# DegardinBruno/Kinetic-GAN

Hardware: AMD Instinct MI355X
Metric: G+D train-step samples/sec, NTU (N,3,64,25) bs=64 at 1/2/4/8 MI355X (higher is better)
Workload: dtype f32; 1 GPU; ntu shapes (N,3,64,25), 60 classes, mlp4, G+D WGAN-GP iteration, 64 samples/GPU; global_batch=64, parallelism=dp1, launch=hipgraph

## Files before the change

include/kgan_hip.h:

```cpp
#ifndef KGAN_HIP_H
#define KGAN_HIP_H

#include <stdint.h>

#ifdef __cplusplus
extern "C" {
#endif

#define KG_ABI_VERSION 9

enum { KG_ACT_NONE = 0, KG_ACT_LRELU = 1, KG_ACT_TANH = 2 };
enum { KG_TAP_TIME = 0,
       KG_TAP_CHANBLOCK = 1  };

int         kg_abi_version(void);
const char* kg_arch(void);
const char* kg_last_error(void);
void        kg_reload_env(void);

typedef struct KgConvGroup {
    const float* x;  int64_t x_sN, x_sC;
    int32_t Cin, T_in, V_in;
    int32_t x_lead;
    const int32_t* vmap;
// ... 58 lines not shown
typedef struct KgWgradReduceJob {
    const float* ws;  float* dw;
    int64_t w_sT, w_sO, w_sI;
    int32_t taps, M, Cin, splits, accumulate;
} KgWgradReduceJob;
#define KG_WGRAD_REDUCE_MAX_JOBS 24
typedef struct KgWgradReduceJobs {
    int32_t njobs;
    KgWgradReduceJob job[KG_WGRAD_REDUCE_MAX_JOBS];
} KgWgradReduceJobs;
int     kg_wgrad_reduce_many(const KgWgradReduceJobs* jobs, void* stream);

int64_t kg_wgrad_many_workspace_bytes(const KgWgradArgs* jobs, int32_t njobs);
int     kg_wgrad_many(const KgWgradArgs* jobs, int32_t njobs, float* ws, int64_t ws_bytes, void* stream);
int     kg_wgrad_many_plan(const KgWgradArgs* jobs, int32_t njobs, int32_t* variant, int32_t* splits);

typedef struct KgAggArgs {
    int32_t N, C, K, V, W;
    int32_t T;
    int32_t rep;
    const float* a;
    const float* x;  int64_t x_sN, x_sC;
    const float* y;  int64_t y_sN, y_sC;
    float* out;  int64_t o_sN, o_sC;
    float* ws;  int64_t ws_bytes;
    int32_t a_transposed;
    int32_t defer_sum;
    const float* res;  int64_t r_sN, r_sC;  int32_t r_T, r_V, r_tstride;  const int32_t* r_inv;
    const float* mask;  int64_t m_sN, m_sC;  float slope;
} KgAggArgs;
// ... 723 lines not shown
```

kinetic-gan_amd/_native.py:

```python
from __future__ import annotations

import ctypes as C
import os
from typing import NamedTuple, Optional, Sequence, Tuple

import torch

_PKG = os.path.dirname(os.path.abspath(__file__))
LIB_PATH = os.environ.get("KG_LIB") or os.path.join(_PKG, "libkgan_hip.so")

ACT_NONE, ACT_LRELU, ACT_TANH = 0, 1, 2
ABI_VERSION = 9
TAP_TIME, TAP_CHANBLOCK = 0, 1

c_f32p = C.c_void_p
c_i32p = C.c_void_p


class _ConvGroup(C.Structure):
    _fields_ = [("x", c_f32p), ("x_sN", C.c_int64), ("x_sC", C.c_int64),
                ("Cin", C.c_int32), ("T_in", C.c_int32), ("V_in", C.c_int32),
                ("x_lead", C.c_int32),
                ("vmap", c_i32p),
                ("w", c_f32p), ("w_sT", C.c_int64), ("w_sO", C.c_int64), ("w_sI", C.c_int64),
# ... 38 lines not shown
class _WgradReduceJob(C.Structure):
    _fields_ = [("ws", c_f32p), ("dw", c_f32p), ("w_sT", C.c_int64), ("w_sO", C.c_int64), ("w_sI", C.c_int64),
                ("taps", C.c_int32), ("M", C.c_int32), ("Cin", C.c_int32), ("splits", C.c_int32),
                ("accumulate", C.c_int32)]


WGRAD_REDUCE_MAX_JOBS = 24
WGRAD_TILE_128x128, WGRAD_TILE_64x64, WGRAD_TILE_64x32, WGRAD_TILE_32x64, WGRAD_TILE_32x32 = 0, 1, 2, 3, 4
WGRAD_TILE_NAMES = {WGRAD_TILE_128x128: "128x128", WGRAD_TILE_64x64: "64x64", WGRAD_TILE_64x32: "64x32",
                    WGRAD_TILE_32x64: "32x64", WGRAD_TILE_32x32: "32x32"}
WGRAD_MAX_SPLITS = 128


class _WgradReduceJobs(C.Structure):
    _fields_ = [("njobs", C.c_int32), ("job", _WgradReduceJob * WGRAD_REDUCE_MAX_JOBS)]


class _AggArgs(C.Structure):
    _fields_ = [("N", C.c_int32), ("C", C.c_int32), ("K", C.c_int32), ("V", C.c_int32), ("W", C.c_int32),
                ("T", C.c_int32), ("rep", C.c_int32),
                ("a", c_f32p),
                ("x", c_f32p), ("x_sN", C.c_int64), ("x_sC", C.c_int64),
                ("y", c_f32p), ("y_sN", C.c_int64), ("y_sC", C.c_int64),
                ("out", c_f32p), ("o_sN", C.c_int64), ("o_sC", C.c_int64),
                ("ws", c_f32p), ("ws_bytes", C.c_int64), ("a_transposed", C.c_int32), ("defer_sum", C.c_int32),
                ("res", c_f32p), ("r_sN", C.c_int64), ("r_sC", C.c_int64), ("r_T", C.c_int32), ("r_V", C.c_int32),
                ("r_tstride", C.c_int32), ("r_inv", c_i32p),
                ("mask", c_f32p), ("m_sN", C.c_int64), ("m_sC", C.c_int64), ("slope", C.c_float)]


# ... 481 lines not shown
    "kg_peak_copy": (C.c_int, [C.c_void_p, C.c_void_p, C.c_int64, C.c_void_p]),
    "kg_conv_workspace_bytes": (C.c_int64, [C.POINTER(_ConvArgs)]),
    "kg_conv_plan_info": (C.c_int, [C.POINTER(_ConvArgs), C.POINTER(C.c_int32), C.POINTER(C.c_int32)]),
    "kg_conv": (C.c_int, [C.POINTER(_ConvArgs), C.c_void_p]),
    "kg_conv_pack_bytes": (C.c_int64, [C.POINTER(_ConvArgs)]),
    "kg_conv_pack": (C.c_int, [C.POINTER(_ConvArgs), C.c_void_p, C.c_int64, C.c_void_p]),
    "kg_conv_many": (C.c_int, [C.POINTER(_ConvArgs), C.c_int32, C.c_void_p]),
    "kg_conv_many_plan": (C.c_int, [C.POINTER(_ConvArgs), C.c_int32, C.POINTER(C.c_int32)]),
    "kg_wgrad_workspace_bytes": (C.c_int64, [C.POINTER(_WgradArgs)]),
    "kg_wgrad": (C.c_int, [C.POINTER(_WgradArgs), C.c_void_p]),
    "kg_wgrad_plan_info": (C.c_int, [C.POINTER(_WgradArgs), C.POINTER(C.c_int32), C.POINTER(C.c_int32)]),
    "kg_wgrad_reduce_many": (C.c_int, [C.POINTER(_WgradReduceJobs), C.c_void_p]),
    "kg_wgrad_many_workspace_bytes": (C.c_int64, [C.POINTER(_WgradArgs), C.c_int32]),
    "kg_wgrad_many": (C.c_int, [C.POINTER(_WgradArgs), C.c_int32, C.c_void_p, C.c_int64, C.c_void_p]),
    "kg_wgrad_many_plan": (C.c_int, [C.POINTER(_WgradArgs), C.c_int32, C.POINTER(C.c_int32), C.POINTER(C.c_int32)]),
    "kg_aggconv_supported": (C.c_int, [C.POINTER(_AggConvArgs)]),
    "kg_aggconv": (C.c_int, [C.POINTER(_AggConvArgs), C.c_void_p]),
    "kg_aggconv_plan_info": (C.c_int, [C.POINTER(_AggConvArgs), C.c_int32, C.POINTER(_AggConvPlanInfo)]),
    "kg_agg_plan_info": (C.c_int, [C.POINTER(_AggArgs), C.c_int32, C.POINTER(_AggPlanInfo)]),
    "kg_agg_outer_many_plan": (C.c_int, [C.POINTER(_AggArgs), C.c_int32, C.POINTER(C.c_int32), C.POINTER(C.c_int32)]),
    "kg_agg_expand": (C.c_int, [C.POINTER(_AggArgs), C.c_void_p]),
    "kg_agg_reduce": (C.c_int, [C.POINTER(_AggArgs), C.c_void_p]),
    "kg_agg_outer_workspace_bytes": (C.c_int64, [C.POINTER(_AggArgs)]),
    "kg_agg_outer": (C.c_int, [C.POINTER(_AggArgs), C.c_void_p]),
    "kg_agg_outer_slabs": (C.c_int, [C.POINTER(_AggArgs)]),
    "kg_agg_outer_many": (C.c_int, [C.POINTER(_AggArgs), C.c_int32, C.c_void_p]),
    "kg_agg_outer_sum_many": (C.c_int, [C.POINTER(_OuterSumJobs), C.c_void_p]),
    "kg_gen_expand": (C.c_int, [C.POINTER(_GenArgs), C.c_void_p]),
    "kg_gen_fold": (C.c_int, [C.POINTER(_GenArgs), C.c_void_p]),
    "kg_gen_adj_finish": (C.c_int, [C.POINTER(_GenAdjJob), C.c_int32, C.c_void_p]),
# ... 81 lines not shown
    "kg_cls_head_workspace_bytes": (C.c_int64, [C.POINTER(_ClsHeadArgs)]),
    "kg_cls_head_fwd": (C.c_int, [C.POINTER(_ClsHeadArgs), C.c_void_p]),
    "kg_cls_head_bwd": (C.c_int, [C.POINTER(_ClsHeadArgs), C.c_void_p]),
    "kg_cls_head_wgrad": (C.c_int, [C.POINTER(_ClsHeadArgs), C.c_void_p]),
    "kg_cls_scores": (C.c_int, [C.POINTER(_ClsScoresArgs), C.c_void_p]),
    "kg_kin_desc_workspace_bytes": (C.c_int64, [C.POINTER(_KinDescArgs)]),
    "kg_kin_desc_lds_bytes": (C.c_int64, [C.POINTER(_KinDescArgs)]),
    "kg_kin_desc": (C.c_int, [C.POINTER(_KinDescArgs), C.c_void_p]),
    "kg_kin_desc_sets_workspace_bytes": (C.c_int64, [C.POINTER(_KinDescSetsArgs)]),
    "kg_kin_desc_sets_lds_bytes": (C.c_int64, [C.POINTER(_KinDescSetsArgs)]),
    "kg_kin_desc_sets": (C.c_int, [C.POINTER(_KinDescSetsArgs), C.c_void_p]),
    "kg_kin_scores_lds_bytes": (C.c_int64, [C.POINTER(_KinScoresArgs)]),
    "kg_kin_scores": (C.c_int, [C.POINTER(_KinScoresArgs), C.c_void_p]),
}

_lib = None


def load_library():
    global _lib
    if _lib is not None:
        return _lib
    if not os.path.exists(LIB_PATH):
        raise RuntimeError(
            f"{LIB_PATH} is missing: run `python -c 'import __graft_entry__ as g; g.build()'` "
            "(hipcc --offload-arch=gfx950). There is no CPU fallback for the st_gcn path.")
    lib = C.CDLL(LIB_PATH)
    for name, (res, args) in EXPORTS.items():
        fn = getattr(lib, name)
        fn.restype = res
        fn.argtypes = args
    if lib.kg_abi_version() != ABI_VERSION:
        raise RuntimeError("libkgan_hip.so ABI version mismatch")
    _lib = lib
    return lib


def _check(rc: int, what: str):
    if rc != 0:
        msg = load_library().kg_last_error().decode()
        raise RuntimeError(f"{what} failed (rc={rc}): {msg}")


# ... 312 lines not shown
    a = _wgrad_args(g, x, Cin, taps, tap_mode, t_stride, vmap, wv, dw, accumulate, extra, keep)
    ws = _workspace("kg_wgrad_workspace_bytes", a, g.device)
    if last_wgrad_plan is not None:
        v, ns = C.c_int32(), C.c_int32()
        _check(lib.kg_wgrad_plan_info(C.byref(a), C.byref(v), C.byref(ns)), "kg_wgrad_plan_info")
        last_wgrad_plan[:] = [(v.value, ns.value)]
    if defer is not None:
        a.defer_reduce = 1
        per = taps * a.M * Cin
        defer.append(dict(ws=ws, dw=dw, w_sT=wv.sT, w_sO=wv.sO, w_sI=wv.sI, taps=taps, M=a.M, Cin=Cin,
                          splits=max(1, ws.numel() // per), accumulate=int(accumulate)))
    _check(lib.kg_wgrad(C.byref(a), _stream()), "kg_wgrad")
    return dw


def wgrad_many(jobs: Sequence[dict]):
    lib = load_library()
    if not jobs:
        return
    arr = (_WgradArgs * len(jobs))()
    keep = []
    for i, j in enumerate(jobs):
        dw = j["out"]
        if not dw.is_contiguous() or dw.dtype != torch.float32:
            raise ValueError("wgrad_many: out must be a contiguous fp32 tensor")
        arr[i] = _wgrad_args(j["g"], j["x"], j["Cin"], j["taps"], j["tap_mode"], j["t_stride"], j.get("vmap"),
                             j["wv"], dw, j.get("accumulate", False), j.get("extra", ()), keep)
    ws = _workspace("kg_wgrad_many_workspace_bytes", arr, jobs[0]["g"].device, len(jobs))
    if last_wgrad_plan is not None:
        v, ns = (C.c_int32 * len(jobs))(), (C.c_int32 * len(jobs))()
        _check(lib.kg_wgrad_many_plan(arr, len(jobs), v, ns), "kg_wgrad_many_plan")
        last_wgrad_plan[:] = list(zip(v, ns))
    _check(lib.kg_wgrad_many(arr, len(jobs), ws.data_ptr(), ws.numel() * 4, _stream()), "kg_wgrad_many")


def wgrad_reduce_many(jobs: list):
    lib = load_library()
    for chunk in _chunks(jobs, WGRAD_REDUCE_MAX_JOBS):
        js = _WgradReduceJobs()
        js.njobs = len(chunk)
        for k, j in enumerate(chunk):
            r = js.job[k]
            r.ws, r.dw = j["ws"].data_ptr(), j["dw"].data_ptr()
            r.w_sT, r.w_sO, r.w_sI = j["w_sT"], j["w_sO"], j["w_sI"]
            r.taps, r.M, r.Cin, r.splits, r.accumulate = j["taps"], j["M"], j["Cin"], j["splits"], j["accumulate"]
        _check(lib.kg_wgrad_reduce_many(C.byref(js), _stream()), "kg_wgrad_reduce_many")
    jobs.clear()

# ... 2166 lines not shown
```

kinetic-gan_amd/csrc/kg_agg.hip:

```cpp
#include <stdlib.h>

#include "kg_common.h"

namespace {

constexpr int NT = 256;

template <int K, int WP>
__device__ __forceinline__ void stage_A(float* As, const float* a, int V, int W, int tr) {
    for (int e = threadIdx.x; e < K * V * WP; e += NT) {
        const int w = e % WP;
        const int kv = e / WP;
        float val = 0.f;
        if (w < W) {
            if (tr) {
                const int k = kv / V, v = kv - k * V;
                val = a[(k * W + w) * V + v];
            } else {
                val = a[kv * W + w];
            }
        }
        As[e] = val;
    }
}
// ... 355 lines not shown
                    int fr = kg_divm(e0, ep.wmul, ep.wshr), w = e0 - fr * W;
                    const int row = (int)r0 + fr;
                    int n = kg_divm(row, ep.tmul, ep.tshr), t = row - n * a.T;
                    const long mbase = (long)c * a.m_sC + r0 * W + e0;
                    if (m4ok) mk[u] = *reinterpret_cast<const f4*>(a.mask + (e0 + 4 <= nfl ? mbase : (long)c * a.m_sC));
#pragma unroll
                    for (int e = 0; e < 4; ++e) {
                        const bool in = e0 + e < nfl;
                        float r = 0.f;
                        if constexpr (RES) {
                            int tb = t, rem = 0;
                            if (a.r_tstride == 2) { tb = t >> 1; rem = t & 1; }
                            else if (a.r_tstride > 2) { tb = t / a.r_tstride; rem = t - tb * a.r_tstride; }
                            const int iv = inv_l[w];
                            const bool hit = in && rem == 0 && tb < a.r_T && iv >= 0;
                            r = a.res[(long)c * a.r_sC + (long)n * a.r_sN + (hit ? tb * a.r_V + iv : 0)];
                            r = hit ? r : 0.f;
                        }
                        rr[u][e] = r;
                        if (MSK && (!m4ok || e0 + 4 > nfl))
                            mk[u][e] = in ? a.mask[(long)c * a.m_sC + (long)n * a.m_sN + (long)t * W + w] : 1.f;
                        if (++w == W) { w = 0; if (++t == a.T) { t = 0; ++n; } }
                    }
                }
#pragma unroll
                for (int u = 0; u < 2; ++u) {
                    if (!live[u]) continue;
                    const int e0 = 4 * (q0 + u * NT);
                    float* dst = a.out + (long)c * a.o_sC + r0 * W + e0;
                    f4 o4;
#pragma unroll
// ... 809 lines not shown
```

kinetic-gan_amd/csrc/kg_wgrad.hip:

```cpp
#include <stdlib.h>

#include <algorithm>
#include <map>
#include <mutex>
#include <vector>

#include "kg_common.h"

namespace {

constexpr int BM = 64, BN = 64, BJ = 64, NT = 256;
#ifndef KG_WGRAD_PJ
#define KG_WGRAD_PJ 64
#endif
constexpr int PJ = KG_WGRAD_PJ;


struct Plan { int tiles_m, tiles_n, splits; int sbeg[4]; int cps[3]; unsigned lmul, lshr, vmul, vshr; int full; };

inline void wg_magic(unsigned d, unsigned& mul, unsigned& shr) {
    mul = 0; shr = 0;
    if (d <= 1) return;
    unsigned lg = 0;
    while ((1u << lg) < d) ++lg;
// ... 63 lines not shown
    if (s > 128) s = 128;
    if (s < 1) s = 1;
    const int per = kg_cdiv(chunks_all, s);
    p.sbeg[0] = 0;
    for (int q = 0; q < 3; ++q) {
        p.cps[q] = per * PJ;
        p.sbeg[q + 1] = p.sbeg[q] + (q < npairs ? kg_cdiv(chunks[q], per) : 0);
    }
    p.splits = p.sbeg[3];
    wg_magic((unsigned)(a->T_out * a->V_out), p.lmul, p.lshr);
    wg_magic((unsigned)a->V_out, p.vmul, p.vshr);
    p.full = (a->M % t.bm == 0 && a->Cin % t.bn == 0) ? 1 : 0;
    return p;
}

template <int GM, int GN, int GK, int WM, int WN, bool SLAB = false>
__device__ __forceinline__ void wgrad_finish(float* const lds, const KgWgradArgs& a, const Plan& p, kg_f32x16 (&acc)[WM][WN],
                                             const int m0, const int c0, const int d, const int split) {
    const int lane = threadIdx.x & 63, wave = threadIdx.x >> 6;
    const int wk = wave / (GM * GN), wmn = wave % (GM * GN);
    const int wm = wmn / GN, wn = wmn % GN;
    if constexpr (GK > 1) {
        float* const red = lds;
        if (wk > 0) {
#pragma unroll
            for (int i = 0; i < WM; ++i)
#pragma unroll
                for (int k = 0; k < WN; ++k)
#pragma unroll
                    for (int r = 0; r < 16; ++r)
// ... 21 lines not shown
#pragma unroll
            for (int r = 0; r < 16; ++r) {
                const int m = m0 + (wm * WM + i) * 32 + (r & 3) + 8 * (r >> 2) + 4 * (lane >> 5);
                if (m < a.M && c < a.Cin) {
                    if (direct) {
                        float* o = a.dw + (long)d * a.w_sT + (long)m * a.w_sO + (long)c * a.w_sI;
                        *o = a.accumulate ? *o + acc[i][k][r] : acc[i][k][r];
                    } else {
                        slab[(long)m * a.Cin + c] = acc[i][k][r];
                    }
                }
            }
        }
}

template <int GM, int GN, int GK, int WM, int WN, int PJ, bool FULL = false, int RW = 1, bool SLAB = false>
__device__ __forceinline__ void wgrad_tile(float* const lds, const KgWgradArgs& a, const Plan& p, const int tile, const int d,
                                           const int split) {
    static_assert(GM * GN * GK == NT / 64, "wave grid");
    constexpr int BM = 32 * GM * WM, BN = 32 * GN * WN;
    constexpr int LDP = PJ + (RW == 1 ? 1 : RW);
    typedef float GsT[BM][LDP];
    typedef float XsT[BN][LDP];
    typedef float FragT __attribute__((ext_vector_type(RW)));
    GsT* const Gs = reinterpret_cast<GsT*>(lds);
    XsT* const Xs = reinterpret_cast<XsT*>(lds + LDS_BUFS * BM * LDP);

    const int tid = threadIdx.x, lane = tid & 63, wave = tid >> 6;
    const int wk = wave / (GM * GN), wmn = wave % (GM * GN);
    const int wm = wmn / GN, wn = wmn % GN;
    const int m0 = (tile / p.tiles_n) * BM;
    const int c0 = (tile % p.tiles_n) * BN;
    const int pr = (split >= p.sbeg[1] ? 1 : 0) + (split >= p.sbeg[2] ? 1 : 0);
    const int pN = pr == 0 ? a.N : a.extra[pr - 1].N;
    const float* const pg = pr == 0 ? a.g : a.extra[pr - 1].g;
    const float* const px_ = pr == 0 ? a.x : a.extra[pr - 1].x;
    const long g_sN = pr == 0 ? a.g_sN : a.extra[pr - 1].g_sN, g_sC = pr == 0 ? a.g_sC : a.extra[pr - 1].g_sC;
    const long x_sN = pr == 0 ? a.x_sN : a.extra[pr - 1].x_sN, x_sC = pr == 0 ? a.x_sC : a.extra[pr - 1].x_sC;
    const int ncols = pN * a.T_out * a.V_out;
    const int L = a.T_out * a.V_out;
    const int cps = p.cps[pr];
    const int jbeg = (split - p.sbeg[pr]) * cps;
    const int jend = min(ncols, jbeg + cps);
    const int shift = (a.tap_mode == KG_TAP_TIME) ? d - (a.taps - 1) / 2 : 0;
    const int choff = (a.tap_mode == KG_TAP_CHANBLOCK) ? d * a.Cin : 0;

    const int cj = tid & (PJ - 1);
    const int r0 = tid / PJ;
    constexpr int RPG = BM / (NT / PJ), RPX = BN / (NT / PJ);
    static_assert(BM % (NT / PJ) == 0 && BN % (NT / PJ) == 0, "staging pattern");

    kg_f32x16 acc[WM][WN];
#pragma unroll
    for (int i = 0; i < WM; ++i)
#pragma unroll
        for (int k = 0; k < WN; ++k)
#pragma unroll
            for (int r = 0; r < 16; ++r) acc[i][k][r] = 0.f;

    float greg[RPG], xreg[RPX];
// ... 35 lines not shown
        for (int i = 0; i < RPG; ++i) pg[i * RSTEP * LDP] = greg[i];
#pragma unroll
        for (int i = 0; i < RPX; ++i) px[i * RSTEP * LDP] = xreg[i];
    };

    if (jbeg < jend) {
        prep(jbeg);
#pragma unroll
        for (int i = 0; i < RPG; ++i) greg[i] = load_g(i);
#pragma unroll
        for (int i = 0; i < RPX; ++i) xreg[i] = load_x(i);
        stash(0);
        __syncthreads();
        int b = 0;
        for (int jc = jbeg; jc < jend; jc += PJ, b ^= (LDS_BUFS - 1)) {
            prep(jc + PJ);
            constexpr int KS = PJ / 2 / GK;
            static_assert(KS % RW == 0, "fragment read width");
            constexpr int KG = KS / RW;
            const float* ga = &Gs[b][wm * 32 * WM + (lane & 31)][RW * (lane >> 5) + 2 * KS * wk];
            const float* xa = &Xs[b][wn * 32 * WN + (lane & 31)][RW * (lane >> 5) + 2 * KS * wk];
            constexpr int LPS = (RPG + RPX + KS / 2 - 1) / (KS / 2);
            FragT av[KG][WM], bv[KG][WN];
            auto read_ab = [&](int q) {
#pragma unroll
                for (int i = 0; i < WM; ++i) av[q][i] = *reinterpret_cast<const FragT*>(ga + i * 32 * LDP + 2 * RW * q);
#pragma unroll
                for (int k = 0; k < WN; ++k) bv[q][k] = *reinterpret_cast<const FragT*>(xa + k * 32 * LDP + 2 * RW * q);
            };
            auto frag = [](const FragT& f, int e) -> float { return f[e]; };
// ... 12 lines not shown
                }
#pragma unroll
                for (int i = 0; i < WM; ++i)
#pragma unroll
                    for (int k = 0; k < WN; ++k)
                        acc[i][k] = __builtin_amdgcn_mfma_f32_32x32x2f32(frag(av[q / RW][i], q % RW), frag(bv[q / RW][k], q % RW),
                                                                         acc[i][k], 0, 0, 0);
                __builtin_amdgcn_sched_barrier(0);
            }
            if constexpr (LDS_BUFS == 1) __syncthreads();
            stash(b ^ (LDS_BUFS - 1));
            __syncthreads();
        }
    }

    wgrad_finish<GM, GN, GK, WM, WN, SLAB>(lds, a, p, acc, m0, c0, d, split);
}

typedef unsigned kg_u32x4 __attribute__((ext_vector_type(4)));
typedef __bf16 kg_bf16x8 __attribute__((ext_vector_type(8)));
typedef __bf16 kg_bf16x2 __attribute__((ext_vector_type(2)));
typedef float kg_f32x2 __attribute__((ext_vector_type(2)));

__device__ __forceinline__ unsigned bs_cvt2(float a, float b) {
    const kg_f32x2 v = {a, b};
    return __builtin_bit_cast(unsigned, __builtin_convertvector(v, kg_bf16x2));
}
__device__ __forceinline__ void bs_split_pair(float x0, float x1, unsigned& h, unsigned& m, unsigned& l) {
    h = bs_cvt2(x0, x1);
    x0 -= __uint_as_float(h << 16); x1 -= __uint_as_float(h & 0xffff0000u);
// ... 169 lines not shown
}

__global__ __launch_bounds__(NT) void kg_wgrad_kernel(const KgWgradArgs a, const Plan p) {
    extern __shared__ float kg_wlds[];
    wgrad_tile<2, 2, 1, 1, 1, PJ, false, RW_S>(kg_wlds, a, p, blockIdx.x, blockIdx.y, blockIdx.z);
}
__global__ __launch_bounds__(NT) void kg_wgrad_bs_kernel(const KgWgradArgs a, const Plan p) {
    extern __shared__ float kg_wlds[];
    wgrad_tile_bs<2, 2, 1, 1, 1, PJ>(kg_wlds, a, p, blockIdx.x, blockIdx.y, blockIdx.z);
}

#ifndef KG_WG_MANY_MAX
#define KG_WG_MANY_MAX 20
#endif
constexpr int MANY_MAX = KG_WG_MANY_MAX;
struct ManyJob { KgWgradArgs a; Plan p; int wg_begin; int variant; };
struct ManyArgs { int njobs; int wg_begin[MANY_MAX];
    ManyJob job[MANY_MAX]; };


template <bool SLAB>
__global__ __launch_bounds__(NT) void kg_wgrad_many_kernel(const ManyArgs m) {
    extern __shared__ float kg_wlds[];
    int ji = 0;
#pragma unroll 1
    while (ji + 1 < m.njobs && (int)blockIdx.x >= m.wg_begin[ji + 1]) ++ji;
    kg_kernarg_warm_at<(int)sizeof(ManyJob), (int)sizeof(ManyArgs)>((unsigned)(offsetof(ManyArgs, job) + ji * sizeof(ManyJob)));
    const ManyJob& j = m.job[ji];
    int local = blockIdx.x - j.wg_begin;
    const int tiles = j.p.tiles_m * j.p.tiles_n;
    const int Q = tiles * j.a.taps, S8 = j.p.splits & ~7;
    int q, split;
    if (local < S8 * Q) {
        const int grp = local / (8 * Q), rem = local - grp * 8 * Q;
        split = grp * 8 + (rem & 7);
        q = rem >> 3;
    } else {
        const int r = j.p.splits - S8, rem = local - S8 * Q;
        split = S8 + rem % r;
        q = rem / r;
    }
    const int tile = q % tiles;
    const int d = q / tiles;
    switch (j.variant) {
        case V_BIG:  wgrad_tile<2, 2, 1, 2, 2, 32, false, RW_B, SLAB>(kg_wlds, j.a, j.p, tile, d, split); break;
        case V_6432: wgrad_tile<2, 1, 2, 1, 1, PJ, false, RW_S, SLAB>(kg_wlds, j.a, j.p, tile, d, split); break;
        case V_3264: wgrad_tile<1, 2, 2, 1, 1, PJ, false, RW_S, SLAB>(kg_wlds, j.a, j.p, tile, d, split); break;
        case V_3232: wgrad_tile<1, 1, 4, 1, 1, PJ_3232, false, RW_S, SLAB>(kg_wlds, j.a, j.p, tile, d, split); break;
        default:     wgrad_tile<2, 2, 1, 1, 1, PJ, false, RW_S, SLAB>(kg_wlds, j.a, j.p, tile, d, split); break;
    }
}

__device__ __forceinline__ void many_locate(const ManyJob& j, int local, int& tile, int& d, int& split) {
    const int tiles = j.p.tiles_m * j.p.tiles_n;
    const int Q = tiles * j.a.taps, S8 = j.p.splits & ~7;
    int q;
    if (local < S8 * Q) {
        const int grp = local / (8 * Q), rem = local - grp * 8 * Q;
        split = grp * 8 + (rem & 7);
        q = rem >> 3;
    } else {
        const int r = j.p.splits - S8, rem = local - S8 * Q;
        split = S8 + rem % r;
        q = rem / r;
// ... 21 lines not shown
}

__global__ __launch_bounds__(256) void kg_wgrad_reduce_kernel(const KgWgradArgs a, int splits) {
    const long per = (long)a.taps * a.M * a.Cin;
    const long i = (long)blockIdx.x * 64 + (threadIdx.x & 63);
    const float s = kg_slab_sum_256(a.ws, per, i, i < per, splits);
    if (i >= per || threadIdx.x >= 64) return;
    const int c = (int)(i % a.Cin);
    const long q = i / a.Cin;
    const int m = (int)(q % a.M);
    const int d = (int)(q / a.M);
    float* o = a.dw + (long)d * a.w_sT + (long)m * a.w_sO + (long)c * a.w_sI;
    *o = a.accumulate ? *o + s : s;
}

struct ReduceBegin { int beg[KG_WGRAD_REDUCE_MAX_JOBS + 1]; };

__host__ __device__ inline bool reduce_vec(const KgWgradReduceJob& j) {
    return (((long)j.taps * j.M * j.Cin) & 3) == 0 && (((unsigned long long)j.ws) & 15ull) == 0;
}

__global__ __launch_bounds__(256) void kg_wgrad_reduce_many_kernel(const KgWgradReduceJobs js, const ReduceBegin rb) {
    typedef float f4 __attribute__((ext_vector_type(4)));
    int ji = 0;
#pragma unroll 1
    while (ji + 1 < js.njobs && (int)blockIdx.x >= rb.beg[ji + 1]) ++ji;
    const KgWgradReduceJob& j = js.job[ji];
    const long per = (long)j.taps * j.M * j.Cin;
    auto store = [&](long i, float s) {
        const int c = (int)(i % j.Cin);
        const long q = i / j.Cin;
        const int m = (int)(q % j.M);
        const int d = (int)(q / j.M);
        float* o = j.dw + (long)d * j.w_sT + (long)m * j.w_sO + (long)c * j.w_sI;
        *o = j.accumulate ? *o + s : s;
    };
    if (reduce_vec(j)) {
        __shared__ f4 red4[4][64];
        const int o = threadIdx.x & 63, sub = threadIdx.x >> 6;
        const long i4 = (long)(blockIdx.x - rb.beg[ji]) * 256 + 4 * o;
        f4 s = {0.f, 0.f, 0.f, 0.f};
        if (i4 < per) {
#pragma unroll 8
            for (int k = sub; k < j.splits; k += 4) s += *reinterpret_cast<const f4*>(j.ws + (long)k * per + i4);
        }
        red4[sub][o] = s;
        __syncthreads();
        if (sub != 0 || i4 >= per) return;
        const f4 t = (red4[0][o] + red4[1][o]) + (red4[2][o] + red4[3][o]);
#pragma unroll
// ... 136 lines not shown
        return 0;
    });
}

extern "C" int64_t kg_wgrad_many_workspace_bytes(const KgWgradArgs* jobs, int32_t njobs) {
    if (jobs == nullptr || njobs < 1) { kg_set_error("kg_wgrad_many: no jobs"); return -1; }
    for (int i = 0; i < njobs; ++i)
        if (validate(&jobs[i]) != 0) return -1;
    const float target = many_cost_target(jobs, njobs);
    int64_t total = 0;
    for (int i = 0; i < njobs; ++i)
        total += (int64_t)many_plan(&jobs[i], target).splits * jobs[i].taps * jobs[i].M * jobs[i].Cin * (int64_t)sizeof(float);
    return total;
}

extern "C" int kg_wgrad_many(const KgWgradArgs* jobs, int32_t njobs, float* ws, int64_t ws_bytes, void* stream) {
    KG_REQUIRE(jobs != nullptr && njobs >= 1, "kg_wgrad_many: no jobs");
    for (int i = 0; i < njobs; ++i) {
        if (int rc = validate(&jobs[i])) return rc;
        KG_REQUIRE(jobs[i].g && jobs[i].x && jobs[i].dw, "kg_wgrad_many: job %d null pointer", i);
        for (int k = 0; k < i; ++k)
            KG_REQUIRE(jobs[k].dw != jobs[i].dw, "kg_wgrad_many: jobs %d and %d write the same dw", k, i);
    }
    static const bool lds_ok = wgrad_lds_attr();
    (void)lds_ok;
    hipStream_t s = (hipStream_t)stream;
    int64_t off = 0;
    KgWgradReduceJobs rj;
    rj.njobs = 0;
    ManyArgs m;
    m.njobs = 0;
    int wgs = 0;
    size_t lds = 0;
    const bool bs = kg_env().wgrad_split != 0;
    auto flush_compute = [&]() -> int {
        if (m.njobs == 0) return 0;
        bool slab = true;
        for (int i = 0; i < m.njobs; ++i) slab = slab && m.job[i].a.defer_reduce != 2;
        if (bs)        hipLaunchKernelGGL(kg_wgrad_many_bs_kernel, dim3(wgs), dim3(NT), lds, s, m);
        else if (slab) hipLaunchKernelGGL(kg_wgrad_many_kernel<true>, dim3(wgs), dim3(NT), lds, s, m);
        else           hipLaunchKernelGGL(kg_wgrad_many_kernel<false>, dim3(wgs), dim3(NT), lds, s, m);
        m.njobs = 0;
        wgs = 0;
        lds = 0;
        return kg_launch_status("kg_wgrad_many");
    };
    auto flush_reduce = [&]() -> int {
        if (rj.njobs == 0) return flush_compute();
        if (int rc = flush_compute()) return rc;
        const int rc = kg_wgrad_reduce_many(&rj, stream);
        rj.njobs = 0;
        return rc;
    };
    if (int rc = many_walk(jobs, njobs, [&](int i, int variant, const Plan& plan) -> int {
        ManyJob& j = m.job[m.njobs];
        j.a = jobs[i];
        j.variant = variant;
        j.p = plan;
        lds = std::max(lds, bs ? tile_lds_bs(j.variant) : tile_lds(j.variant));
        const int64_t bytes = (int64_t)j.p.splits * j.a.taps * j.a.M * j.a.Cin * (int64_t)sizeof(float);
        KG_REQUIRE(ws != nullptr && off + bytes <= ws_bytes, "kg_wgrad_many: workspace %ld < %ld bytes", (long)ws_bytes,
                   (long)(off + bytes));
        j.a.ws = ws + off / (int64_t)sizeof(float);
        j.a.ws_bytes = bytes;
        off += bytes;
        j.wg_begin = wgs;
        m.wg_begin[m.njobs] = wgs;
        wgs += j.p.tiles_m * j.p.tiles_n * j.a.taps * j.p.splits;
        if (j.p.splits == 1) {
            j.a.defer_reduce = 2;
        } else {
            j.a.defer_reduce = 1;
            KgWgradReduceJob& r = rj.job[rj.njobs++];
            r.ws = j.a.ws; r.dw = j.a.dw;
            r.w_sT = j.a.w_sT; r.w_sO = j.a.w_sO; r.w_sI = j.a.w_sI;
            r.taps = j.a.taps; r.M = j.a.M; r.Cin = j.a.Cin; r.splits = j.p.splits; r.accumulate = j.a.accumulate;
        }
        if (++m.njobs == MANY_MAX)
            if (int rc = flush_compute()) return rc;
        if (rj.njobs == KG_WGRAD_REDUCE_MAX_JOBS)
            if (int rc = flush_reduce()) return rc;
        return 0;
    })) return rc;
    return flush_reduce();
}


extern "C" int kg_wgrad_reduce_many(const KgWgradReduceJobs* jobs, void* stream) {
    KG_REQUIRE(jobs != nullptr, "kg_wgrad_reduce_many: null jobs");
    KG_REQUIRE(jobs->njobs >= 1 && jobs->njobs <= KG_WGRAD_REDUCE_MAX_JOBS, "kg_wgrad_reduce_many: njobs=%d", jobs->njobs);
    ReduceBegin rb;
    rb.beg[0] = 0;
    for (int i = 0; i < jobs->njobs; ++i) {
        const KgWgradReduceJob& j = jobs->job[i];
        KG_REQUIRE(j.ws && j.dw && j.taps >= 1 && j.M >= 1 && j.Cin >= 1 && j.splits >= 1,
                   "kg_wgrad_reduce_many: job %d is malformed", i);
        const long per = (long)j.taps * j.M * j.Cin;
        rb.beg[i + 1] = rb.beg[i] + kg_cdiv(per, reduce_vec(j) ? 256 : 64);
        for (int k = 0; k < i; ++k)
            KG_REQUIRE(jobs->job[k].dw != j.dw, "kg_wgrad_reduce_many: jobs %d and %d write the same dw", k, i);
    }
    hipLaunchKernelGGL(kg_wgrad_reduce_many_kernel, dim3(rb.beg[jobs->njobs]), dim3(256), 0, (hipStream_t)stream, *jobs,
                       rb);
    return kg_launch_status("kg_wgrad_reduce_many");
}
```

kinetic-gan_amd/ops.py:

```python
from __future__ import annotations

import os
from dataclasses import dataclass
from typing import Optional, Tuple

import torch
from torch.autograd import Function
from torch.autograd.function import once_differentiable

from . import _native as nv
from ._native import ACT_LRELU, ACT_NONE, ACT_TANH, TAP_CHANBLOCK, TAP_TIME, Group, WView

_SKIP_PARAM_GRADS = False


class no_param_grads:
    def __enter__(self):
        global _SKIP_PARAM_GRADS
        self.prev = _SKIP_PARAM_GRADS
        _SKIP_PARAM_GRADS = True

    def __exit__(self, *exc):
        global _SKIP_PARAM_GRADS
        _SKIP_PARAM_GRADS = self.prev


class _ParamSink:
    def __init__(self):
        self.views = {}
        self.enabled = True
        self.use_side_stream = False
        self.side = {}
        self.dirty = set()
        self.defer = True
        self.pending = {}
        self.pending_rows = []

    def stream(self, device):
        st = self.side.get(device)
        if st is None:
            st = self.side[device] = torch.cuda.Stream(device=device)
        return st


_SINK = _ParamSink()
if os.environ.get("KG_PARAM_SINK") == "0":
    _SINK.enabled = False
if os.environ.get("KG_PARAM_SIDE_STREAM") == "1":
    _SINK.use_side_stream = True
if os.environ.get("KG_PARAM_DEFER") == "0":
    _SINK.defer = False


def register_param_sink(param: torch.Tensor, flat_view: torch.Tensor):
    assert flat_view.numel() == param.numel() and flat_view.is_contiguous()
    key = (param.data_ptr(), param.numel())
    _SINK.views[key] = flat_view
    return key


def unregister_param_sinks(keys):
    for k in keys:
        _SINK.views.pop(k, None)


def clear_param_sinks():
    _SINK.views.clear()


def param_sink_options(enabled: Optional[bool] = None, side_stream: Optional[bool] = None,
                       defer: Optional[bool] = None):
    if enabled is not None:
        _SINK.enabled = enabled
    if side_stream is not None:
        _SINK.use_side_stream = side_stream
    if defer is not None:
        _SINK.defer = defer


def _sink_of(t: Optional[torch.Tensor]):
    if t is None or not _SINK.enabled or not _SINK.views:
        return None
    return _SINK.views.get((t.data_ptr(), t.numel()))


class _on_side:
# ... 14 lines not shown
            self.ctx.__enter__()
        return self

    def __exit__(self, *exc):
        if self.ctx is not None:
            self.ctx.__exit__(*exc)


def _wgrad_job(view, spec, pairs):
    (x0, g0), rest = pairs[0], pairs[1:]
    return dict(g=g0, x=x0, Cin=spec.Cin, taps=spec.taps, tap_mode=spec.tap_mode, t_stride=spec.t_stride,
                vmap=spec.vmap, wv=WView(spec.wv.sT, spec.wv.sO, spec.wv.sI), out=view, accumulate=True,
                extra=[(g, x) for x, g in rest])


def join_param_sink():
    pending, _SINK.pending = _SINK.pending, {}
    flush_outer()
    with torch.no_grad():
        entries = list(pending.values())
        rnd = 0
        while True:
            jobs = [_wgrad_job(view, spec, pairs[3 * rnd:3 * rnd + 3]) for (view, spec, pairs) in entries
                    if pairs[3 * rnd:3 * rnd + 3]]
            if not jobs:
                break
            with _on_side(*[t for j in jobs for t in (j["g"], j["x"])]):
                nv.wgrad_many(jobs)
            rnd += 1
        rows, _SINK.pending_rows = _SINK.pending_rows, []
        while rows:
            seen, now, later = set(), [], []
            for views, g, y in rows:
                ptrs = [v.data_ptr() for v in views]
                if any(p in seen for p in ptrs):
                    later.append((views, g, y))
                else:
                    seen.update(ptrs)
                    now.append(dict(x=g, y=y, out=views[0], out2=views[1] if len(views) > 1 else None,
                                    accumulate=True))
            with _on_side(*[t for j in now for t in (j["x"], j["y"]) if t is not None]):
                nv.rowsum_many(now)
            rows = later
    for dev in list(_SINK.dirty):
        torch.cuda.current_stream(dev).wait_stream(_SINK.side[dev])
# ... 676 lines not shown
```

Baseline: 20740 samples/s.

## Fold bias-gradient row sums into the batched wgrad kernel

```diff
diff --git a/include/kgan_hip.h b/include/kgan_hip.h
--- a/include/kgan_hip.h
+++ b/include/kgan_hip.h
@@ -96,6 +96,17 @@
 int64_t kg_wgrad_many_workspace_bytes(const KgWgradArgs* jobs, int32_t njobs);
 int     kg_wgrad_many(const KgWgradArgs* jobs, int32_t njobs, float* ws, int64_t ws_bytes, void* stream);
 int     kg_wgrad_many_plan(const KgWgradArgs* jobs, int32_t njobs, int32_t* variant, int32_t* splits);
+
+typedef struct KgWgradBiasReq {
+    int32_t job;
+    int32_t pair_mask;
+    float*  db;
+    float*  db2;
+    int32_t accumulate;
+} KgWgradBiasReq;
+int64_t kg_wgrad_many_bias_workspace_bytes(const KgWgradArgs* jobs, int32_t njobs, const KgWgradBiasReq* reqs, int32_t nreqs);
+int     kg_wgrad_many_bias(const KgWgradArgs* jobs, int32_t njobs, const KgWgradBiasReq* reqs, int32_t nreqs, float* ws,
+                           int64_t ws_bytes, void* stream);
 
 typedef struct KgAggArgs {
     int32_t N, C, K, V, W;
diff --git a/kinetic-gan_amd/_native.py b/kinetic-gan_amd/_native.py
--- a/kinetic-gan_amd/_native.py
+++ b/kinetic-gan_amd/_native.py
@@ -76,6 +76,10 @@
 
 class _WgradReduceJobs(C.Structure):
     _fields_ = [("njobs", C.c_int32), ("job", _WgradReduceJob * WGRAD_REDUCE_MAX_JOBS)]
+
+
+class _WgradBiasReq(C.Structure):
+    _fields_ = [("job", C.c_int32), ("pair_mask", C.c_int32), ("db", c_f32p), ("db2", c_f32p), ("accumulate", C.c_int32)]
 
 
 class _AggArgs(C.Structure):
@@ -587,6 +591,9 @@
     "kg_wgrad_many_workspace_bytes": (C.c_int64, [C.POINTER(_WgradArgs), C.c_int32]),
     "kg_wgrad_many": (C.c_int, [C.POINTER(_WgradArgs), C.c_int32, C.c_void_p, C.c_int64, C.c_void_p]),
     "kg_wgrad_many_plan": (C.c_int, [C.POINTER(_WgradArgs), C.c_int32, C.POINTER(C.c_int32), C.POINTER(C.c_int32)]),
+    "kg_wgrad_many_bias_workspace_bytes": (C.c_int64, [C.POINTER(_WgradArgs), C.c_int32, C.POINTER(_WgradBiasReq), C.c_int32]),
+    "kg_wgrad_many_bias": (C.c_int, [C.POINTER(_WgradArgs), C.c_int32, C.POINTER(_WgradBiasReq), C.c_int32, C.c_void_p, C.c_int64,
+                                      C.c_void_p]),
     "kg_aggconv_supported": (C.c_int, [C.POINTER(_AggConvArgs)]),
     "kg_aggconv": (C.c_int, [C.POINTER(_AggConvArgs), C.c_void_p]),
     "kg_aggconv_plan_info": (C.c_int, [C.POINTER(_AggConvArgs), C.c_int32, C.POINTER(_AggConvPlanInfo)]),
@@ -698,6 +705,8 @@
     "kg_kin_scores": (C.c_int, [C.POINTER(_KinScoresArgs), C.c_void_p]),
 }
 
+ADDITIVE_EXPORTS = ("kg_wgrad_many_bias_workspace_bytes", "kg_wgrad_many_bias")
+
 _lib = None
 
 
@@ -711,6 +720,8 @@
             "(hipcc --offload-arch=gfx950). There is no CPU fallback for the st_gcn path.")
     lib = C.CDLL(LIB_PATH)
     for name, (res, args) in EXPORTS.items():
+        if name in ADDITIVE_EXPORTS and not hasattr(lib, name):
+            continue
         fn = getattr(lib, name)
         fn.restype = res
         fn.argtypes = args
@@ -1053,9 +1064,15 @@
     return dw
 
 
-def wgrad_many(jobs: Sequence[dict]):
+def wgrad_many_bias_supported() -> bool:
+    return all(hasattr(load_library(), name) for name in ADDITIVE_EXPORTS)
+
+
+def wgrad_many(jobs: Sequence[dict], bias: Sequence[dict] = ()):
     lib = load_library()
     if not jobs:
+        if bias:
+            raise ValueError("wgrad_many: bias requests without jobs")
         return
     arr = (_WgradArgs * len(jobs))()
     keep = []
@@ -1065,12 +1082,29 @@
             raise ValueError("wgrad_many: out must be a contiguous fp32 tensor")
         arr[i] = _wgrad_args(j["g"], j["x"], j["Cin"], j["taps"], j["tap_mode"], j["t_stride"], j.get("vmap"),
                              j["wv"], dw, j.get("accumulate", False), j.get("extra", ()), keep)
-    ws = _workspace("kg_wgrad_many_workspace_bytes", arr, jobs[0]["g"].device, len(jobs))
     if last_wgrad_plan is not None:
         v, ns = (C.c_int32 * len(jobs))(), (C.c_int32 * len(jobs))()
         _check(lib.kg_wgrad_many_plan(arr, len(jobs), v, ns), "kg_wgrad_many_plan")
         last_wgrad_plan[:] = list(zip(v, ns))
-    _check(lib.kg_wgrad_many(arr, len(jobs), ws.data_ptr(), ws.numel() * 4, _stream()), "kg_wgrad_many")
+    if not bias:
+        ws = _workspace("kg_wgrad_many_workspace_bytes", arr, jobs[0]["g"].device, len(jobs))
+        _check(lib.kg_wgrad_many(arr, len(jobs), ws.data_ptr(), ws.numel() * 4, _stream()), "kg_wgrad_many")
+        return
+    if not wgrad_many_bias_supported():
+        raise RuntimeError("wgrad_many: this libkgan_hip.so has no kg_wgrad_many_bias")
+    reqs = (_WgradBiasReq * len(bias))()
+    for r, b in zip(reqs, bias):
+        M = arr[b["job"]].M if 0 <= b["job"] < len(jobs) else -1
+        for o in (b["out"], b.get("out2")):
+            if o is not None:
+                _need_cuda(_dest(o, M, "wgrad_many: bias destinations must be contiguous fp32 vectors of M elements"))
+        r.job, r.pair_mask, r.accumulate = b["job"], b["pairs"], int(bool(b.get("accumulate", False)))
+        r.db, r.db2 = b["out"].data_ptr(), _ptr(b.get("out2"))
+    nbytes = lib.kg_wgrad_many_bias_workspace_bytes(arr, len(jobs), reqs, len(bias))
+    if nbytes < 0:
+        _check(-1, "kg_wgrad_many_bias_workspace_bytes")
+    ws = torch.empty(max(1, nbytes // 4), dtype=torch.float32, device=jobs[0]["g"].device)
+    _check(lib.kg_wgrad_many_bias(arr, len(jobs), reqs, len(bias), ws.data_ptr(), ws.numel() * 4, _stream()), "kg_wgrad_many_bias")
 
 
 def wgrad_reduce_many(jobs: list):
diff --git a/kinetic-gan_amd/csrc/kg_agg.hip b/kinetic-gan_amd/csrc/kg_agg.hip
--- a/kinetic-gan_amd/csrc/kg_agg.hip
+++ b/kinetic-gan_amd/csrc/kg_agg.hip
@@ -393,7 +393,7 @@
                             else if (a.r_tstride > 2) { tb = t / a.r_tstride; rem = t - tb * a.r_tstride; }
                             const int iv = inv_l[w];
                             const bool hit = in && rem == 0 && tb < a.r_T && iv >= 0;
-                            r = a.res[(long)c * a.r_sC + (long)n * a.r_sN + (hit ? tb * a.r_V + iv : 0)];
+                            r = a.res[(long)c * a.r_sC + (hit ? (long)n * a.r_sN + tb * a.r_V + iv : 0)];
                             r = hit ? r : 0.f;
                         }
                         rr[u][e] = r;
diff --git a/kinetic-gan_amd/csrc/kg_wgrad.hip b/kinetic-gan_amd/csrc/kg_wgrad.hip
--- a/kinetic-gan_amd/csrc/kg_wgrad.hip
+++ b/kinetic-gan_amd/csrc/kg_wgrad.hip
@@ -101,6 +101,8 @@
     return p;
 }
 
+struct ManyBias { float* out; int mask; int accumulate; };
+
 template <int GM, int GN, int GK, int WM, int WN, bool SLAB = false>
 __device__ __forceinline__ void wgrad_finish(float* const lds, const KgWgradArgs& a, const Plan& p, kg_f32x16 (&acc)[WM][WN],
                                              const int m0, const int c0, const int d, const int split) {
@@ -152,9 +154,9 @@
         }
 }
 
-template <int GM, int GN, int GK, int WM, int WN, int PJ, bool FULL = false, int RW = 1, bool SLAB = false>
+template <int GM, int GN, int GK, int WM, int WN, int PJ, bool FULL = false, int RW = 1, bool SLAB = false, bool BIAS = false>
 __device__ __forceinline__ void wgrad_tile(float* const lds, const KgWgradArgs& a, const Plan& p, const int tile, const int d,
-                                           const int split) {
+                                           const int split, const ManyBias& bz = ManyBias()) {
     static_assert(GM * GN * GK == NT / 64, "wave grid");
     constexpr int BM = 32 * GM * WM, BN = 32 * GN * WN;
     constexpr int LDP = PJ + (RW == 1 ? 1 : RW);
@@ -182,6 +184,9 @@
     const int jend = min(ncols, jbeg + cps);
     const int shift = (a.tap_mode == KG_TAP_TIME) ? d - (a.taps - 1) / 2 : 0;
     const int choff = (a.tap_mode == KG_TAP_CHANBLOCK) ? d * a.Cin : 0;
+    bool carry = false;
+    if constexpr (BIAS) carry = d == 0 && c0 == 0 && ((bz.mask >> pr) & 1) != 0;
+    float bsum = 0.f;
 
     const int cj = tid & (PJ - 1);
     const int r0 = tid / PJ;
@@ -247,6 +252,19 @@
         __syncthreads();
         int b = 0;
         for (int jc = jbeg; jc < jend; jc += PJ, b ^= (LDS_BUFS - 1)) {
+            if constexpr (BIAS) {
+                if (carry && tid < BM) {
+                    const FragT* const row = reinterpret_cast<const FragT*>(&Gs[b][tid][0]);
+#pragma unroll
+                    for (int k = 0; k < PJ / RW; ++k) {
+                        const FragT v = row[k];
+                        float t = v[0];
+#pragma unroll
+                        for (int e = 1; e < RW; ++e) t += v[e];
+                        bsum += t;
+                    }
+                }
+            }
             prep(jc + PJ);
             constexpr int KS = PJ / 2 / GK;
             static_assert(KS % RW == 0, "fragment read width");
@@ -289,6 +307,14 @@
         }
     }
 
+    if constexpr (BIAS) {
+        if (carry && tid < BM && m0 + tid < a.M) {
+            const int m = m0 + tid;
+            const int skip = ((bz.mask & 1) || pr < 1 ? 0 : p.sbeg[1]) + ((bz.mask & 2) || pr < 2 ? 0 : p.sbeg[2] - p.sbeg[1]);
+            float* const o = bz.out + ((long)(split - skip) * a.M + m);
+            *o = bz.accumulate ? *o + bsum : bsum;
+        }
+    }
     wgrad_finish<GM, GN, GK, WM, WN, SLAB>(lds, a, p, acc, m0, c0, d, split);
 }
 
@@ -488,7 +514,7 @@
 #define KG_WG_MANY_MAX 20
 #endif
 constexpr int MANY_MAX = KG_WG_MANY_MAX;
-struct ManyJob { KgWgradArgs a; Plan p; int wg_begin; int variant; };
+struct ManyJob { KgWgradArgs a; Plan p; int wg_begin; int variant; ManyBias b; };
 struct ManyArgs { int njobs; int wg_begin[MANY_MAX];
     ManyJob job[MANY_MAX]; };
 
@@ -517,11 +543,11 @@
     const int tile = q % tiles;
     const int d = q / tiles;
     switch (j.variant) {
-        case V_BIG:  wgrad_tile<2, 2, 1, 2, 2, 32, false, RW_B, SLAB>(kg_wlds, j.a, j.p, tile, d, split); break;
-        case V_6432: wgrad_tile<2, 1, 2, 1, 1, PJ, false, RW_S, SLAB>(kg_wlds, j.a, j.p, tile, d, split); break;
-        case V_3264: wgrad_tile<1, 2, 2, 1, 1, PJ, false, RW_S, SLAB>(kg_wlds, j.a, j.p, tile, d, split); break;
-        case V_3232: wgrad_tile<1, 1, 4, 1, 1, PJ_3232, false, RW_S, SLAB>(kg_wlds, j.a, j.p, tile, d, split); break;
-        default:     wgrad_tile<2, 2, 1, 1, 1, PJ, false, RW_S, SLAB>(kg_wlds, j.a, j.p, tile, d, split); break;
+        case V_BIG:  wgrad_tile<2, 2, 1, 2, 2, 32, false, RW_B, SLAB, true>(kg_wlds, j.a, j.p, tile, d, split, j.b); break;
+        case V_6432: wgrad_tile<2, 1, 2, 1, 1, PJ, false, RW_S, SLAB, true>(kg_wlds, j.a, j.p, tile, d, split, j.b); break;
+        case V_3264: wgrad_tile<1, 2, 2, 1, 1, PJ, false, RW_S, SLAB, true>(kg_wlds, j.a, j.p, tile, d, split, j.b); break;
+        case V_3232: wgrad_tile<1, 1, 4, 1, 1, PJ_3232, false, RW_S, SLAB, true>(kg_wlds, j.a, j.p, tile, d, split, j.b); break;
+        default:     wgrad_tile<2, 2, 1, 1, 1, PJ, false, RW_S, SLAB, true>(kg_wlds, j.a, j.p, tile, d, split, j.b); break;
     }
 }
 
@@ -573,26 +599,35 @@
     *o = a.accumulate ? *o + s : s;
 }
 
-struct ReduceBegin { int beg[KG_WGRAD_REDUCE_MAX_JOBS + 1]; };
+constexpr int REDUCE_MAX = 2 * MANY_MAX > KG_WGRAD_REDUCE_MAX_JOBS ? 2 * MANY_MAX : KG_WGRAD_REDUCE_MAX_JOBS;
+struct RJob { KgWgradReduceJob j; float* dw2; };
+struct RJobs { int njobs; RJob job[REDUCE_MAX]; };
+struct ReduceBegin { int beg[REDUCE_MAX + 1]; };
 
 __host__ __device__ inline bool reduce_vec(const KgWgradReduceJob& j) {
     return (((long)j.taps * j.M * j.Cin) & 3) == 0 && (((unsigned long long)j.ws) & 15ull) == 0;
 }
 
-__global__ __launch_bounds__(256) void kg_wgrad_reduce_many_kernel(const KgWgradReduceJobs js, const ReduceBegin rb) {
+__global__ __launch_bounds__(256) void kg_wgrad_reduce_many_kernel(const RJobs js, const ReduceBegin rb) {
     typedef float f4 __attribute__((ext_vector_type(4)));
     int ji = 0;
 #pragma unroll 1
     while (ji + 1 < js.njobs && (int)blockIdx.x >= rb.beg[ji + 1]) ++ji;
-    const KgWgradReduceJob& j = js.job[ji];
+    const KgWgradReduceJob& j = js.job[ji].j;
+    float* const dw2 = js.job[ji].dw2;
     const long per = (long)j.taps * j.M * j.Cin;
     auto store = [&](long i, float s) {
         const int c = (int)(i % j.Cin);
         const long q = i / j.Cin;
         const int m = (int)(q % j.M);
         const int d = (int)(q / j.M);
-        float* o = j.dw + (long)d * j.w_sT + (long)m * j.w_sO + (long)c * j.w_sI;
+        const long at = (long)d * j.w_sT + (long)m * j.w_sO + (long)c * j.w_sI;
+        float* o = j.dw + at;
         *o = j.accumulate ? *o + s : s;
+        if (dw2) {
+            o = dw2 + at;
+            *o = j.accumulate ? *o + s : s;
+        }
     };
     if (reduce_vec(j)) {
         __shared__ f4 red4[4][64];
@@ -759,7 +794,51 @@
     return total;
 }
 
-extern "C" int kg_wgrad_many(const KgWgradArgs* jobs, int32_t njobs, float* ws, int64_t ws_bytes, void* stream) {
+
+namespace {
+
+int reduce_launch(const RJobs& js, void* stream) {
+    ReduceBegin rb;
+    rb.beg[0] = 0;
+    for (int i = 0; i < js.njobs; ++i) {
+        const KgWgradReduceJob& j = js.job[i].j;
+        KG_REQUIRE(j.ws && j.dw && j.taps >= 1 && j.M >= 1 && j.Cin >= 1 && j.splits >= 1,
+                   "kg_wgrad_reduce_many: job %d is malformed", i);
+        const long per = (long)j.taps * j.M * j.Cin;
+        rb.beg[i + 1] = rb.beg[i] + kg_cdiv(per, reduce_vec(j) ? 256 : 64);
+        for (int k = 0; k < i; ++k)
+            KG_REQUIRE(js.job[k].j.dw != j.dw, "kg_wgrad_reduce_many: jobs %d and %d write the same dw", k, i);
+    }
+    hipLaunchKernelGGL(kg_wgrad_reduce_many_kernel, dim3(rb.beg[js.njobs]), dim3(256), 0, (hipStream_t)stream, js, rb);
+    return kg_launch_status("kg_wgrad_reduce_many");
+}
+
+inline int bias_entries(const Plan& p, int mask) {
+    int n = 0;
+    for (int q = 0; q < 3; ++q)
+        if ((mask >> q) & 1) n += p.sbeg[q + 1] - p.sbeg[q];
+    return n;
+}
+inline int64_t bias_slab_bytes(const Plan& p, int mask, int M) {
+    return (((int64_t)bias_entries(p, mask) * M * (int64_t)sizeof(float)) + 15) & ~(int64_t)15;
+}
+
+int validate_bias(const KgWgradArgs* jobs, int njobs, const KgWgradBiasReq* reqs, int nreqs, int* of_job) {
+    for (int i = 0; i < njobs; ++i) of_job[i] = -1;
+    KG_REQUIRE(nreqs >= 0 && (nreqs == 0 || reqs != nullptr), "kg_wgrad_many_bias: %d requests without a table", nreqs);
+    for (int r = 0; r < nreqs; ++r) {
+        const KgWgradBiasReq& b = reqs[r];
+        KG_REQUIRE(b.job >= 0 && b.job < njobs, "kg_wgrad_many_bias: request %d names job %d of %d", r, b.job, njobs);
+        KG_REQUIRE(of_job[b.job] < 0, "kg_wgrad_many_bias: requests %d and %d name job %d", of_job[b.job], r, b.job);
+        KG_REQUIRE(b.pair_mask > 0 && b.pair_mask < (1 << (1 + jobs[b.job].nextra)),
+                   "kg_wgrad_many_bias: request %d pair_mask=%d, job %d has %d pairs", r, b.pair_mask, b.job, 1 + jobs[b.job].nextra);
+        of_job[b.job] = r;
+    }
+    return 0;
+}
+
+int many_launch(const KgWgradArgs* jobs, int32_t njobs, const KgWgradBiasReq* reqs, int32_t nreqs, float* ws, int64_t ws_bytes,
+                void* stream) {
     KG_REQUIRE(jobs != nullptr && njobs >= 1, "kg_wgrad_many: no jobs");
     for (int i = 0; i < njobs; ++i) {
         if (int rc = validate(&jobs[i])) return rc;
@@ -767,17 +846,29 @@
         for (int k = 0; k < i; ++k)
             KG_REQUIRE(jobs[k].dw != jobs[i].dw, "kg_wgrad_many: jobs %d and %d write the same dw", k, i);
     }
+    std::vector<int> of_job(njobs);
+    if (int rc = validate_bias(jobs, njobs, reqs, nreqs, of_job.data())) return rc;
+    for (int r = 0; r < nreqs; ++r) {
+        KG_REQUIRE(reqs[r].db != nullptr && reqs[r].db != reqs[r].db2, "kg_wgrad_many_bias: request %d destinations", r);
+        for (int k = 0; k < r; ++k)
+            for (const float* d : {reqs[k].db, reqs[k].db2})
+                KG_REQUIRE(d == nullptr || (d != reqs[r].db && d != reqs[r].db2),
+                           "kg_wgrad_many_bias: requests %d and %d write the same destination", k, r);
+    }
     static const bool lds_ok = wgrad_lds_attr();
     (void)lds_ok;
     hipStream_t s = (hipStream_t)stream;
     int64_t off = 0;
-    KgWgradReduceJobs rj;
+    int64_t top = ws_bytes;
+    if (nreqs > 0 && ws != nullptr) top -= (int64_t)(((unsigned long long)ws + (unsigned long long)ws_bytes) & 15ull);
+    RJobs rj;
     rj.njobs = 0;
     ManyArgs m;
     m.njobs = 0;
     int wgs = 0;
     size_t lds = 0;
     const bool bs = kg_env().wgrad_split != 0;
+    KG_REQUIRE(!bs || nreqs == 0, "kg_wgrad_many_bias: the bf16-split tiles (KG_WGRAD_SPLIT=1) carry no bias sums");
     auto flush_compute = [&]() -> int {
         if (m.njobs == 0) return 0;
         bool slab = true;
@@ -793,7 +884,7 @@
     auto flush_reduce = [&]() -> int {
         if (rj.njobs == 0) return flush_compute();
         if (int rc = flush_compute()) return rc;
-        const int rc = kg_wgrad_reduce_many(&rj, stream);
+        const int rc = reduce_launch(rj, stream);
         rj.njobs = 0;
         return rc;
     };
@@ -804,8 +895,8 @@
         j.p = plan;
         lds = std::max(lds, bs ? tile_lds_bs(j.variant) : tile_lds(j.variant));
         const int64_t bytes = (int64_t)j.p.splits * j.a.taps * j.a.M * j.a.Cin * (int64_t)sizeof(float);
-        KG_REQUIRE(ws != nullptr && off + bytes <= ws_bytes, "kg_wgrad_many: workspace %ld < %ld bytes", (long)ws_bytes,
-                   (long)(off + bytes));
+        KG_REQUIRE(ws != nullptr && off + bytes <= top, "kg_wgrad_many: workspace %ld < %ld bytes", (long)ws_bytes,
+                   (long)(off + bytes + (ws_bytes - top)));
         j.a.ws = ws + off / (int64_t)sizeof(float);
         j.a.ws_bytes = bytes;
         off += bytes;
@@ -816,36 +907,77 @@
             j.a.defer_reduce = 2;
         } else {
             j.a.defer_reduce = 1;
-            KgWgradReduceJob& r = rj.job[rj.njobs++];
+            RJob& rr = rj.job[rj.njobs++];
+            KgWgradReduceJob& r = rr.j;
+            rr.dw2 = nullptr;
             r.ws = j.a.ws; r.dw = j.a.dw;
             r.w_sT = j.a.w_sT; r.w_sO = j.a.w_sO; r.w_sI = j.a.w_sI;
             r.taps = j.a.taps; r.M = j.a.M; r.Cin = j.a.Cin; r.splits = j.p.splits; r.accumulate = j.a.accumulate;
         }
+        j.b = ManyBias{nullptr, 0, 0};
+        if (of_job[i] >= 0) {
+            const KgWgradBiasReq& b = reqs[of_job[i]];
+            j.b.mask = b.pair_mask;
+            if (j.p.splits == 1 && b.db2 == nullptr) {
+                j.b.out = b.db;
+                j.b.accumulate = b.accumulate;
+            } else {
+                const int64_t bb = bias_slab_bytes(j.p, b.pair_mask, j.a.M);
+                KG_REQUIRE(off + bb <= top, "kg_wgrad_many_bias: workspace %ld bytes: no room for the bias slab of job %d",
+                           (long)ws_bytes, i);
+                top -= bb;
+                j.b.out = ws + top / (int64_t)sizeof(float);
+                RJob& rr = rj.job[rj.njobs++];
+                KgWgradReduceJob& r = rr.j;
+                rr.dw2 = b.db2;
+                r.ws = j.b.out; r.dw = b.db;
+                r.w_sT = 0; r.w_sO = 1; r.w_sI = 0;
+                r.taps = 1; r.M = j.a.M; r.Cin = 1; r.splits = bias_entries(j.p, b.pair_mask); r.accumulate = b.accumulate;
+            }
+        }
         if (++m.njobs == MANY_MAX)
             if (int rc = flush_compute()) return rc;
-        if (rj.njobs == KG_WGRAD_REDUCE_MAX_JOBS)
+        if (rj.njobs + 2 > REDUCE_MAX)
             if (int rc = flush_reduce()) return rc;
         return 0;
     })) return rc;
     return flush_reduce();
 }
 
+}
+
+extern "C" int kg_wgrad_many(const KgWgradArgs* jobs, int32_t njobs, float* ws, int64_t ws_bytes, void* stream) {
+    return many_launch(jobs, njobs, nullptr, 0, ws, ws_bytes, stream);
+}
+
+extern "C" int64_t kg_wgrad_many_bias_workspace_bytes(const KgWgradArgs* jobs, int32_t njobs, const KgWgradBiasReq* reqs,
+                                                      int32_t nreqs) {
+    int64_t total = kg_wgrad_many_workspace_bytes(jobs, njobs);
+    if (total < 0) return -1;
+    std::vector<int> of_job(njobs);
+    if (validate_bias(jobs, njobs, reqs, nreqs, of_job.data()) != 0) return -1;
+    if (nreqs == 0) return total;
+    total = (total + 15) & ~(int64_t)15;
+    many_walk(jobs, njobs, [&](int i, int, const Plan& p) -> int {
+        if (of_job[i] >= 0 && (p.splits > 1 || reqs[of_job[i]].db2)) total += bias_slab_bytes(p, reqs[of_job[i]].pair_mask, jobs[i].M);
+        return 0;
+    });
+    return total + 16;
+}
+
+extern "C" int kg_wgrad_many_bias(const KgWgradArgs* jobs, int32_t njobs, const KgWgradBiasReq* reqs, int32_t nreqs, float* ws,
+                                  int64_t ws_bytes, void* stream) {
+    return many_launch(jobs, njobs, reqs, nreqs, ws, ws_bytes, stream);
+}
 
 extern "C" int kg_wgrad_reduce_many(const KgWgradReduceJobs* jobs, void* stream) {
     KG_REQUIRE(jobs != nullptr, "kg_wgrad_reduce_many: null jobs");
     KG_REQUIRE(jobs->njobs >= 1 && jobs->njobs <= KG_WGRAD_REDUCE_MAX_JOBS, "kg_wgrad_reduce_many: njobs=%d", jobs->njobs);
-    ReduceBegin rb;
-    rb.beg[0] = 0;
+    RJobs js;
+    js.njobs = jobs->njobs;
     for (int i = 0; i < jobs->njobs; ++i) {
-        const KgWgradReduceJob& j = jobs->job[i];
-        KG_REQUIRE(j.ws && j.dw && j.taps >= 1 && j.M >= 1 && j.Cin >= 1 && j.splits >= 1,
-                   "kg_wgrad_reduce_many: job %d is malformed", i);
-        const long per = (long)j.taps * j.M * j.Cin;
-        rb.beg[i + 1] = rb.beg[i] + kg_cdiv(per, reduce_vec(j) ? 256 : 64);
-        for (int k = 0; k < i; ++k)
-            KG_REQUIRE(jobs->job[k].dw != j.dw, "kg_wgrad_reduce_many: jobs %d and %d write the same dw", k, i);
-    }
-    hipLaunchKernelGGL(kg_wgrad_reduce_many_kernel, dim3(rb.beg[jobs->njobs]), dim3(256), 0, (hipStream_t)stream, *jobs,
-                       rb);
-    return kg_launch_status("kg_wgrad_reduce_many");
-}
+        js.job[i].j = jobs->job[i];
+        js.job[i].dw2 = nullptr;
+    }
+    return reduce_launch(js, stream);
+}
diff --git a/kinetic-gan_amd/ops.py b/kinetic-gan_amd/ops.py
--- a/kinetic-gan_amd/ops.py
+++ b/kinetic-gan_amd/ops.py
@@ -35,6 +35,8 @@
         self.defer = True
         self.pending = {}
         self.pending_rows = []
+        self.bias_in_wgrad = True
+        self.bias_record = None
 
     def stream(self, device):
         st = self.side.get(device)
@@ -50,6 +52,9 @@
     _SINK.use_side_stream = True
 if os.environ.get("KG_PARAM_DEFER") == "0":
     _SINK.defer = False
+if os.environ.get("KG_WGRAD_BIAS") == "0":
+    _SINK.bias_in_wgrad = False
+_NV_WGRAD_MANY = nv.wgrad_many
 
 
 def register_param_sink(param: torch.Tensor, flat_view: torch.Tensor):
@@ -69,7 +74,9 @@
 
 
 def param_sink_options(enabled: Optional[bool] = None, side_stream: Optional[bool] = None,
-                       defer: Optional[bool] = None):
+                       defer: Optional[bool] = None, bias_in_wgrad: Optional[bool] = None):
+    if bias_in_wgrad is not None:
+        _SINK.bias_in_wgrad = bias_in_wgrad
     if enabled is not None:
         _SINK.enabled = enabled
     if side_stream is not None:
@@ -114,21 +121,72 @@
                 extra=[(g, x) for x, g in rest])
 
 
+def _wgrad_bias_route() -> bool:
+    return (_SINK.bias_in_wgrad and nv.wgrad_many is _NV_WGRAD_MANY and os.environ.get("KG_WGRAD_SPLIT", "0") == "0"
+            and nv.wgrad_many_bias_supported())
+
+
+def _same_view(a, b) -> bool:
+    return a.data_ptr() == b.data_ptr() and a.shape == b.shape and a.stride() == b.stride() and a.dtype == b.dtype
+
+
+def _attach_bias(jobs, rows):
+    reqs, rest, served, taken = [], [], set(), set()
+    for views, g, y in rows:
+        ptrs = [v.data_ptr() for v in views]
+        hit = None
+        if y is None and 1 <= len(views) <= 2 and len(set(ptrs)) == len(ptrs) and not any(p in served for p in ptrs):
+            for ji, job in enumerate(jobs):
+                if ji in taken or any(v.numel() != job["g"].shape[1] for v in views):
+                    continue
+                for pi, pg in enumerate([job["g"]] + [ge for ge, _ in job["extra"]]):
+                    if _same_view(pg, g):
+                        hit = (ji, pi)
+                        break
+                if hit:
+                    break
+        if hit is None:
+            rest.append((views, g, y))
+            continue
+        taken.add(hit[0])
+        served.update(ptrs)
+        reqs.append(dict(job=hit[0], pairs=1 << hit[1], out=views[0], out2=views[1] if len(views) > 1 else None,
+                         accumulate=True))
+    return reqs, rest
+
+
 def join_param_sink():
     pending, _SINK.pending = _SINK.pending, {}
     flush_outer()
     with torch.no_grad():
         entries = list(pending.values())
-        rnd = 0
+        rows, _SINK.pending_rows = _SINK.pending_rows, []
+        rounds, rnd = [], 0
         while True:
             jobs = [_wgrad_job(view, spec, pairs[3 * rnd:3 * rnd + 3]) for (view, spec, pairs) in entries
                     if pairs[3 * rnd:3 * rnd + 3]]
             if not jobs:
                 break
+            rounds.append(jobs)
+            rnd += 1
+        riding, left = [[] for _ in rounds], rows
+        if rows and _wgrad_bias_route():
+            for k, jobs in enumerate(rounds):
+                riding[k], left = _attach_bias(jobs, left)
+            if left:
+                riding, left = [[] for _ in rounds], rows
+        rows = left
+        for jobs, reqs in zip(rounds, riding):
+            if _SINK.bias_record is not None:
+                _SINK.bias_record += [("wgrad", [v for v in (r["out"], r["out2"]) if v is not None], jobs[r["job"]]["g"], None)
+                                      for r in reqs]
             with _on_side(*[t for j in jobs for t in (j["g"], j["x"])]):
-                nv.wgrad_many(jobs)
-            rnd += 1
-        rows, _SINK.pending_rows = _SINK.pending_rows, []
+                if reqs:
+                    nv.wgrad_many(jobs, bias=reqs)
+                else:
+                    nv.wgrad_many(jobs)
+        if _SINK.bias_record is not None:
+            _SINK.bias_record += [("rowsum", list(views), g, y) for views, g, y in rows]
         while rows:
             seen, now, later = set(), [], []
             for views, g, y in rows:
```

Measured after the change: 20900 samples/s (median of 6 runs). Within noise of the previous version (+0.8%).
